# leonsick/depthg

Measured on AMD Instinct MI355X. Metric: correlation-loss steps/sec at B=32,C=384,28x28 (fwd+bwd, per-GPU batch 32), higher is better.
Workload: dtype bf16 (feats) / f16 (code) MFMA inputs, f32 accumulate

## Files before the change

### depthg_amd/_lib.py

```python
import ctypes
import os

_HERE = os.path.dirname(os.path.abspath(__file__))
LIB_PATH = os.environ.get("DEPTHG_LIB") or os.path.join(_HERE, "lib", "libdepthg_hip.so")

DG_OUT_COUNT = 9
DG_OUT_TOTAL = 8
DG_VERSION = 118
DG_POINTWISE, DG_ZERO_CLAMP, DG_STABALIZE, DG_DEPTH_TERM, DG_NEED_GRAD, DG_SHARED_COORDS, DG_IDENTITY_GRID, DG_LINE_GRID, \
    DG_EXACT_MASKS, DG_FEATS_UNIT = (1 << i for i in range(10))
DG_LIN_LAYERNORM, DG_LIN_GELU, DG_LIN_IN_BF16, DG_LIN_OUT_BF16 = 1, 2, 4, 8

class CorrDesc(ctypes.Structure):
    _fields_ = [("B", ctypes.c_int32), ("C", ctypes.c_int32), ("D", ctypes.c_int32), ("h", ctypes.c_int32),
                ("w", ctypes.c_int32), ("S", ctypes.c_int32), ("n_neg", ctypes.c_int32),
                ("depth_h", ctypes.c_int32), ("depth_w", ctypes.c_int32), ("flags", ctypes.c_uint32),
                ("shift_intra", ctypes.c_float), ("shift_inter", ctypes.c_float), ("shift_neg", ctypes.c_float),
                ("shift_depth", ctypes.c_float),
                ("w_intra", ctypes.c_float), ("w_inter", ctypes.c_float), ("w_neg", ctypes.c_float),
                ("w_depth", ctypes.c_float), ("code_h", ctypes.c_int32), ("code_w", ctypes.c_int32)]


class AdamSeg(ctypes.Structure):
    _fields_ = [("param", ctypes.c_void_p), ("grad", ctypes.c_void_p), ("exp_avg", ctypes.c_void_p), ("exp_avg_sq", ctypes.c_void_p),
# ... 84 lines not shown
    "dg_vit_linear_forward": (_I, [vp, vp, vp, f32, vp, vp, vp, vp] + [i32] * 4 + [vp]),
    "dg_depthenc_workspace_bytes": (_SZ, [i32] * 5),
    "dg_depthenc_forward": (_I, [vp] * 12 + [i32] * 8 + [vp, vp, _SZ, vp]),
    "dg_depthenc_backward": (_I, [vp] * 12 + [i32] * 6 + [vp] * 11 + [_SZ, vp]),
    "dg_xattn_workspace_bytes": (_SZ, [i32] * 5),
    "dg_xattn_forward": (_I, [vp] * 3 + [i32] * 5 + [f32, f32, u64, vp, vp, vp, _SZ, vp]),
    "dg_xattn_backward": (_I, [vp] * 6 + [i32] * 5 + [f32, f32, u64, vp, vp, vp, vp, _SZ, vp]),
    "dg_xattn_keep_mask": (_I, [u64] + [i32] * 4 + [f32, vp, vp]),
    "dg_augment_workspace_bytes": (_SZ, [i32] * 3),
    "dg_augment_forward": (_I, [vp] + [i64] * 4 + [vp] * 4 + [i32] * 6 + [vp, vp, vp, _SZ, vp]),
    "dg_batch_prep": (_I, [vp, _SZ, vp, vp, vp] + [i32] * 4 + [vp] * 7),
    "dg_corr_main_kernel_name": (_STR, [cp]),
    "dg_corr_intra_folded": (_I, [cp]),
    "dg_prof_main_span": (_I, [vp]),
    "dg_corr_relaunch_main": (_I, [cp, vp, vp, _SZ, vp]),
}
EXPORTS = list(SIGNATURES)

_lib = None


def load():
    global _lib
    if _lib is not None:
        return _lib
    if not os.path.exists(LIB_PATH):
        raise RuntimeError(
            f"depthg_amd: {LIB_PATH} not found. Build it with `make -C depthg_amd/csrc` "
            "(or `python -c 'import __graft_entry__ as g; g.build()'`). There is no fallback path.")
    lib = ctypes.CDLL(LIB_PATH)
# ... 16 lines not shown
```

### depthg_amd/csrc/dg_api_corr.hip

```cpp
#include "dg_api.h"
#include "dg_corr_args.h"
#include "dg_taps.h"

static unsigned long long* g_prof_span = nullptr;
extern "C" int dg_prof_main_span(void* span) { g_prof_span = static_cast<unsigned long long*>(span); return DG_OK; }

enum class Prep { Small, Dense, General };
enum class Sampler { Plane, ChannelLast };
enum class MainKernel { Small, Corr2, CorrMain };
enum class Depth { None, Job, GsBlocks, GsOwnLaunch };
enum class Hist { Rows, Blobs };
enum class Masks { None, Sampled, DenseRaw, DenseSplit };

struct PairSet {
    int rop;
    int op;
    int neg;
    bool mapped;
    float shift;
    int slot_loss, slot_cd;
    float fin_scale;
    int gidx, csel, dest;
    float factor;
};
// ... 31 lines not shown
    int8_t gr_key[DG_MAX_JOBS], gr_first[DG_MAX_JOBS];
    int32_t gr_nblk[DG_MAX_JOBS];
    size_t nhwc_f[2], nhwc_c[2];
    size_t rows_f[DG_MAX_NEG + 2], rows_c[DG_MAX_NEG + 2];
    size_t op[DG_MAX_NEG + 2], inv[DG_MAX_NEG + 2], colpart[DG_MAX_NEG + 2], bbar[DG_MAX_NEG + 2];
    size_t ccolpart[DG_MAX_NEG + 2], csum[DG_MAX_NEG + 2], bsplit[DG_MAX_NEG + 2];
    size_t rvec[DG_MAX_NEG + 2], rimg[DG_MAX_NEG + 2];
    size_t nz, nzsum;
    size_t dRA[DG_MAX_NEG + 3], dRB[DG_MAX_NEG + 2];
    size_t part[DG_MAX_NEG + 3];
    size_t comb[2], scratch_out, taps, gbuf[DG_MAX_NEG + 2];
    size_t ticket;
    size_t maskbits[DG_MAX_NEG + 2];
    size_t clo[2];
    size_t gr_list, gr_count, gr_rank;
    size_t dRA2[DG_MAX_NEG + 2], dRBs[DG_MAX_NEG + 2], dRB2[DG_MAX_NEG + 2][2], dRBm[DG_MAX_NEG + 2], part4, om;
    size_t total;

    bool small() const { return prep == Prep::Small; }
    bool dense() const { return prep == Prep::Dense; }
    bool plane() const { return sampler == Sampler::Plane; }
    bool has_masks() const { return masks != Masks::None; }
    bool depth_in_gs() const { return depth_run == Depth::GsBlocks || depth_run == Depth::GsOwnLaunch; }
    bool dense_masks() const { return masks == Masks::DenseRaw || masks == Masks::DenseSplit; }
    bool intra_symmetric() const { return !pointwise || fold; }
    const int64_t* batch_map(int k, const int64_t* perms) const {
        return k < 0 ? nullptr : reinterpret_cast<const int64_t*>(reinterpret_cast<uintptr_t>(perms) + (size_t)k * B * sizeof(int64_t));
    }
    const int64_t* map_of(int t, const int64_t* perms) const { return batch_map(ps[t].mapped ? ps[t].neg : -1, perms); }
};
// ... 141 lines not shown
    if ((d->flags & DG_EXACT_MASKS) && p.grad && (d->flags & DG_ZERO_CLAMP) && !xmask && !xmask_dense && !p.small())
        return fail(DG_ERR_UNSUPPORTED, "DG_EXACT_MASKS: exact clamp masks exist on small sample grids (always on there) and on the dense "
                                        "identity grid with C <= 384 (padded to 384), D <= 80, P >= 160, B <= 64, zero_clamp without stabalize");
    p.masks = xmask ? Masks::Sampled : (!xmask_dense ? Masks::None : (p.pointwise ? Masks::DenseSplit : Masks::DenseRaw));
    for (int t = 0; t < p.T; ++t) p.maskbits[t] = take(p.has_masks() ? B * (size_t)(p.Ppad / 32) * p.Ppad * 4 : 0);
    p.main = p.small() ? MainKernel::Small
                       : (p.grad && dg_corr2_shape_supported(p.KF, p.KD, p.D, p.lo, p.hi, p.Ppad, p.B) ? MainKernel::Corr2 : MainKernel::CorrMain);
    static const bool fold_on = [] { const char* e = getenv("DG_FOLD_INTRA"); return !(e && e[0] == '0'); }();
    p.fold = fold_on && p.main == MainKernel::Corr2 && p.pointwise && !xmask;
    p.half = p.main == MainKernel::Corr2 && ident && p.N * p.B <= 512 && p.S == p.h && p.S == p.w;
    p.depth_run = (!p.depth || p.small()) ? Depth::None : (!p.grad ? Depth::Job : (p.dense_masks() ? Depth::GsOwnLaunch : Depth::GsBlocks));
    for (int i = 0; i < 2; ++i) p.clo[i] = take(p.masks == Masks::DenseSplit ? B * (size_t)(p.Ppad / 32) * p.KD * 64 : 0);
    p.gr_list = take((size_t)DG_MAX_JOBS * B * DG_GR_CAP * 4);
    p.gr_count = take((size_t)DG_MAX_JOBS * B * 4);
    p.gr_rank = take((size_t)DG_MAX_JOBS * B * 2);
    {
        const bool sg = p.small() && p.grad, two = sg && p.pointwise;
        const size_t gt = B * p.Ppad * p.KD * 4;
        for (int t = 0; t < p.T; ++t) {
            p.dRA2[t] = take(two ? gt : 0);
            p.dRBs[t] = take(sg && p.nsplit == 2 ? gt : 0);
            for (int k = 0; k < 2; ++k) p.dRB2[t][k] = take(two && k < p.nsplit ? gt : 0);
            p.dRBm[t] = take(sg && t >= 2 && (p.pointwise || p.nsplit == 2) ? gt : 0);
        }
        p.part4 = take(p.small() ? (size_t)(p.T + 1) * B * p.nsplit * 16 : 0);
        p.om = take(p.small() ? (size_t)(p.T + 1) * 4 : 0);
    }
    if (intra_feats) {
        const int x = p.xop = p.T;
        p.nhwc_x = take(rows ? 0 : B * HW * p.C4 * 4);
// ... 341 lines not shown
        f.ext_inv = c.feat_inv ? c.feat_inv + (size_t)o * p.B * p.P : nullptr;
        f.K = p.C; f.K4 = p.C4; f.Kpad = p.KF; f.is_code = 0; f.h = p.h; f.w = p.w;
        DgGatherJob& k = g.jobs[nj++];
        k.src = p.plane() ? f32(c.ws, p.rows_c[o]) : f32(c.ws, p.nhwc_c[srcsel]); k.coords = c.coords(o); k.srcidx = idx;
        k.blob = c.ws + p.op[o]; k.inv_norm = f32(c.ws, p.inv[o]); k.colpart = f32(c.ws, p.ccolpart[o]);
        k.K = p.D; k.K4 = p.D4; k.Kpad = p.KD; k.is_code = 1; k.h = p.hc; k.w = p.wc;
    }
    g.njobs = nj;
    g.direct = p.plane() ? 1 : 0;
    if (p.masks == Masks::Sampled) cd_mask_args(c, p.rows_c, g.cd);
    g.pre = pre_late;
    DG_HIP(dg_launch_gather(g, p.KF, c.stream));
    return DG_OK;
}

static int fwd_colmeans(Fwd& c) {
    const Plan& p = c.p;
    const DgCorrArgs& a = c.a;
    DgColmeanArgs m;
    memset(&m, 0, sizeof(m));
    m.nops = p.nopx(); m.B = p.B; m.P = p.P; m.Ppad = p.Ppad; m.KF = p.KF; m.KD = p.KD;
    for (int o = 0; o < p.nopx(); ++o) {
        m.colpart[o] = p.pointwise ? f32(c.ws, p.colpart[o]) : nullptr; m.bbar[o] = f32(c.ws, p.bbar[o]);
        m.bsplit[o] = reinterpret_cast<__bf16*>(c.ws + p.bsplit[o]);
        m.ngroups[o] = p.Ppad / 32;
        m.ccolpart[o] = f32(c.ws, p.ccolpart[o]); m.csum[o] = f32(c.ws, p.csum[o]);
    }
    m.zero_word = p.depth_in_gs() ? reinterpret_cast<unsigned int*>(c.ws + p.ticket) : nullptr;
    m.zero_words9 = a.wctr;
    if (p.gr_on) {
        m.gr.nh = p.T; m.gr.nkeys = p.gr_nkeys; m.gr.B = p.B;
        for (int t = 0; t < p.T; ++t) { m.gr.sidx[t] = p.map_of(t, c.perms); m.gr.key[t] = p.gr_key[t]; }
        m.gr.list = reinterpret_cast<int32_t*>(c.ws + p.gr_list); m.gr.count = reinterpret_cast<int32_t*>(c.ws + p.gr_count);
        m.gr.rank = reinterpret_cast<int16_t*>(c.ws + p.gr_rank);
    }
    if (p.dense() && p.pointwise) {
        m.dc.code[0] = c.code; m.dc.code[1] = c.code_pos;
        for (int o = 0; o < 2; ++o) { m.dc.blob[o] = c.ws + p.op[o]; m.dc.inv_norm[o] = f32(c.ws, p.inv[o]); m.dc.ccolpart[o] = f32(c.ws, p.ccolpart[o]); }
        m.dc.B = p.B; m.dc.D = p.D; m.dc.KF = p.KF; m.dc.KD = p.KD; m.dc.h = p.h; m.dc.w = p.w; m.dc.P = p.P; m.dc.Ppad = p.Ppad;
        if (p.masks == Masks::DenseSplit) { m.dc.clo[0] = c.ws + p.clo[0]; m.dc.clo[1] = c.ws + p.clo[1]; }
    }
    if (c.split) {
        DgColmeanArgs ms = m;
        ms.zsel = 1; m.zsel = 2;
        DG_HIP(c.side->hand_over(0));
        DG_HIP(dg_launch_colmean(ms, c.side->stream()));
    }
    DG_HIP(dg_launch_colmean(m, c.stream));
    return DG_OK;
}
// ... 219 lines not shown
                f.add(k == 0 ? p.dRB[t] : p.dRBs[t], route, q.gidx, q.csel, q.factor, q.dest, 0);
                if (p.pointwise) f.add(p.dRB2[t][k], route, q.gidx, q.csel, q.factor, q.dest, 0, 0, om);
            }
        }
    }
}

static void scatter_sources_blobs(const Plan& p, const int64_t* perms, ScatterFill& f) {
    const int hf = p.half ? 1 : 0;
    for (int t = 0; t < p.T; ++t) {
        const PairSet& q = p.ps[t];
        const bool doubled = t == 0 && p.intra_symmetric();
        f.add(p.dRA[t], nullptr, q.gidx, 0, doubled ? 2.0f * q.factor : q.factor, 0, 1, hf);
        if (!doubled) f.add(p.dRB[t], p.batch_map(q.neg, perms), q.gidx, q.csel, q.factor, q.dest, 0, hf);
    }
}

static int corr_backward_impl(const dg_corr_desc* desc, const float* grad_scalars, const float* grad_total, const float* coords1,
                              const float* coords2, const int64_t* perms, float* grad_code, float* grad_code_pos,
                              void* workspace, size_t workspace_bytes, dg_stream_t stream_) {
    Plan p{};
    int rc = make_plan(desc, p);
    if (rc != DG_OK) return rc;
    if (!p.grad) return fail(DG_ERR_INVALID, "dg_corr_backward needs a descriptor with DG_NEED_GRAD (as used in forward)");
    if (!coords1 || !coords2 || !grad_code || !grad_code_pos || !workspace) return fail(DG_ERR_INVALID, "null pointer");
    if (p.N > 0 && !perms) return fail(DG_ERR_INVALID, "perms is null with n_neg=%d", p.N);
    if (workspace_bytes < p.total) return fail(DG_ERR_WORKSPACE, "workspace %zu < required %zu bytes", workspace_bytes, p.total);
    char* ws = static_cast<char*>(workspace);
    DgScatterArgs s;
    memset(&s, 0, sizeof(s));
    ScatterFill fill{s, ws};
    if (p.small()) scatter_sources_small(p, perms, fill);
    else scatter_sources_blobs(p, perms, fill);
    if (p.depth) fill.add(p.dRA[p.T], nullptr, 3, 0, 2.0f * p.grad_f, 0, 1);
    s.coords1 = coords1; s.coords2 = coords2; s.gscal = grad_scalars; s.gtot = grad_total;
    s.wtot[0] = desc->w_intra; s.wtot[1] = desc->w_inter; s.wtot[2] = desc->w_neg; s.wtot[3] = desc->w_depth;
    s.comb[0] = f32(ws, p.comb[0]); s.comb[1] = f32(ws, p.comb[1]);
    s.taps = ws + p.taps;
    s.xop = ws + p.op[0]; s.xinv = f32(ws, p.inv[0]); s.blob_bytes = p.blob; s.blob_off_c = p.blob_off_c;
    s.xinv_dest[0] = f32(ws, p.inv[0]); s.xinv_dest[1] = p.nops > 1 ? f32(ws, p.inv[1]) : nullptr;
    s.out[0] = grad_code; s.out[1] = grad_code_pos;
    s.B = p.B; s.D = p.D; s.DP = p.KD; s.h = p.hc; s.w = p.wc; s.S = p.S; s.Sh = p.Sh; s.P = p.P; s.Ppad = p.Ppad;
    if ((size_t)p.hc * p.wc > 4096) return fail(DG_ERR_UNSUPPORTED, "code map %dx%d too large for the gradient gather (max 4096 pixels)", p.hc, p.wc);
    s.DC = 8;
    s.dense = p.dense() ? 1 : 0;
    s.taps_ready = p.dense() ? 0 : 1;
    DG_HIP(dg_launch_scatter(s, static_cast<hipStream_t>(stream_)));
    return DG_OK;
}

extern "C" int dg_corr_backward(const dg_corr_desc* desc, const float* grad_scalars, const float* coords1,
                                const float* coords2, const int64_t* perms, float* grad_code, float* grad_code_pos,
                                void* workspace, size_t workspace_bytes, dg_stream_t stream_) {
    if (!grad_scalars) return fail(DG_ERR_INVALID, "null pointer");
    return corr_backward_impl(desc, grad_scalars, nullptr, coords1, coords2, perms, grad_code, grad_code_pos, workspace,
                              workspace_bytes, stream_);
}

extern "C" int dg_corr_backward_total(const dg_corr_desc* desc, const float* grad_total, const float* coords1,
                                      const float* coords2, const int64_t* perms, float* grad_code, float* grad_code_pos,
// ... 91 lines not shown
    if (!workspace || workspace_bytes < p.total) return fail(DG_ERR_WORKSPACE, "workspace missing or too small");
    if (p.N > 0 && !perms) return fail(DG_ERR_INVALID, "perms is null");
    char* ws = static_cast<char*>(workspace);
    if (p.small()) {
        DgSmallArgs m;
        small_args(p, desc, ws, perms, m);
        m.out = f32(ws, p.scratch_out);
        DG_HIP(dg_launch_corr_small(m, static_cast<hipStream_t>(stream_)));
        return DG_OK;
    }
    DgCorrArgs a;
    build_corr_jobs(p, ws, perms, a);
    return launch_main(p, a, static_cast<hipStream_t>(stream_));
}

extern "C" int dg_corr_intra_folded(const dg_corr_desc* desc) {
    Plan p{};
    if (make_plan(desc, p) != DG_OK) return -1;
    return p.fold ? 1 : 0;
}

extern "C" const char* dg_corr_main_kernel_name(const dg_corr_desc* desc) {
    Plan p{};
    if (make_plan(desc, p) != DG_OK) return nullptr;
    return p.main == MainKernel::Small ? "k_corr_small" : (p.main == MainKernel::Corr2 ? "k_corr2" : "k_corr_main");
}

extern "C" int dg_normalize_split(int32_t B, int32_t C, int32_t h, int32_t w, const float* src, int32_t nchunks, int32_t chunk_c,
                                  float* const* dst, dg_stream_t stream_) {
    if (B < 1 || C < 1 || h < 1 || w < 1 || !src || !dst) return fail(DG_ERR_INVALID, "dg_normalize_split: bad arguments");
// ... 7 lines not shown
```

### depthg_amd/csrc/dg_corr_args.h

```cpp
#pragma once
#include "dg_device.h"

__host__ __device__ inline int dg_perm32(int pl) {
    int s = pl >> 4, u = (pl >> 3) & 1, hh = (pl >> 2) & 1, v = pl & 3;
    return (2 * s + hh) * 8 + 4 * u + v;
}

#ifndef DG_F_IG
#define DG_F_IG 4
#endif
__host__ __device__ inline int dg_f_off(int q, int g) {
    constexpr int IG = DG_F_IG;
    return ((g / IG) * 32 + q) * (IG * 16) + (((g % IG) ^ ((q / (16 / IG)) % IG)) * 16);
}

struct DgBlob {
    int GF, GD, KD;
    int off_c, off_p, bytes;
    __host__ __device__ DgBlob(int KF, int KD_) : GF(KF / 8), GD(KD_ / 8), KD(KD_) {
        off_c = 32 * GF * 16;
        off_p = off_c + GD * 32 * 16;
        bytes = off_p + 4 * KD * 16;
    }
    __host__ __device__ int f(int q, int g) const { return dg_f_off(q, g); }
// ... 9 lines not shown
    static constexpr int BYTES = OFF_P + 4 * KD * 16;
    static constexpr int CHUNKS = BYTES / 1024;
    static constexpr int CHUNK_C0 = OFF_C / 1024;
    static constexpr int CHUNK_P0 = OFF_P / 1024;
    static_assert(BYTES % 1024 == 0 && OFF_C % 1024 == 0 && OFF_P % 1024 == 0, "blob parts must be KiB multiples");
    static_assert(GF % 16 == 0, "swizzle needs 16-granule groups");
};

__host__ __device__ inline size_t dg_gtile_off(int p, int d, int DP) {
    const int q = p & 31;
    return ((size_t)(p >> 5) * (DP >> 5) + (d >> 5)) * 1024 + (q >> 3) * 256 + ((d & 31) + 32 * ((q >> 2) & 1)) * 4 + (q & 3);
}

#define DG_XROWS_LDS (4 * 33 * 16)
template <int NDF>
__device__ __forceinline__ void dg_load_code_rows(const char* Cp, char* T, int lane, _Float16 (&x)[NDF][16]) {
        const int r = lane & 31, h = lane >> 5;
    i32x4 raw[NDF][2];
#pragma unroll
    for (int f = 0; f < NDF; ++f)
#pragma unroll
        for (int k = 0; k < 2; ++k) raw[f][k] = *reinterpret_cast<const i32x4*>(Cp + f * 2048 + k * 1024 + lane * 16);
#pragma unroll
    for (int f = 0; f < NDF; ++f) {
#pragma unroll
        for (int k = 0; k < 2; ++k) {
            const int L = k * 64 + lane;
            *reinterpret_cast<i32x4*>(T + ((L >> 5) * 33 + (L & 31)) * 16) = raw[f][k];
        }
#pragma unroll
        for (int i = 0; i < 16; ++i) {
            const int q = (i & 3) + 8 * (i >> 2) + 4 * h;
            x[f][i] = *reinterpret_cast<const _Float16*>(T + ((r >> 3) * 33 + q) * 16 + (r & 7) * 2);
        }
    }
}

enum { DG_JOB_HELPER = 0, DG_JOB_DEPTH = 1 };

struct DgJob {
    const char* Rop;
    const char* Sop;
    const float* rvec;
    const float* rimg;
    const uint32_t* maskbits;
    const float* nzR;
    const float* nzS;
    const float* RcInv;
    const float* Scsum;
    const int64_t* ridx;
// ... 267 lines not shown
    int cnt = 0;
#pragma unroll
    for (int j = 0; j < DG_MAX_JOBS; ++j) {
        const bool hit = src[j] == m;
        const unsigned long long mask = __ballot(hit);
        if (hit) {
            const int rk = cnt + __popcll(mask & ((1ull << lane) - 1ull));
            g.rank[j * B + lane] = (int16_t)(rk < 32767 ? rk : 32767);
            if (rk < DG_GR_CAP) g.list[(key * B + m) * DG_GR_CAP + rk] = j | (lane << 8);
        }
        cnt += __popcll(mask);
    }
    if (lane == 0) g.count[key * B + m] = cnt < DG_GR_CAP ? cnt : DG_GR_CAP;
}

struct DgColmeanArgs {
    const float* colpart[DG_MAX_NEG + 2];
    float* bbar[DG_MAX_NEG + 2];
    __bf16* bsplit[DG_MAX_NEG + 2];
    const float* ccolpart[DG_MAX_NEG + 2];
    float* csum[DG_MAX_NEG + 2];
    int32_t ngroups[DG_MAX_NEG + 2];
    int32_t nops, B, P, Ppad, KF, KD;
    unsigned int* zero_word;
    unsigned int* zero_words9;
    DgGroupArgs gr;
    DgDenseCodeArgs dc;
    int32_t zsel;
};

struct DgRowmeanJob {
    const char* A;
    const float* bbar;
    const __bf16* bsplit;
    const int64_t* aidx;
    const int64_t* bidx;
    float* rvec;
    float* rimg;
};
struct DgRowmeanArgs {
    DgRowmeanJob jobs[DG_MAX_NEG + 2];
// ... 25 lines not shown
    int32_t nsrc;
    const float* coords1;
    const float* coords2;
    const float* gscal;
    const float* gtot;
    float wtot[4];
    float* comb[2];
    char* taps;
    const char* xop;
    const float* xinv;
    const float* xinv_dest[2];
    int32_t blob_bytes, blob_off_c;
    float* out[2];
    int32_t B, D, DP, h, w, S, Sh, P, Ppad, DC;
    int32_t dense;
    int8_t craw[2][DG_MAX_SCATTER / 2], cfin[2][DG_MAX_SCATTER / 2];
    int8_t ncraw[2], ncfin[2];
    int8_t crawh[2][DG_MAX_SCATTER / 2], cfinh[2][DG_MAX_SCATTER / 2];
    int8_t ncrawh[2], ncfinh[2];
    int32_t routed_half;
    int32_t taps_ready;
    int32_t naxpy;
    float* axo[DG_MAX_NEG + 2];
    const float* axd[DG_MAX_NEG + 2];
    const float* axd2[DG_MAX_NEG + 2];
    const float* axs[DG_MAX_NEG + 2];
    const float* axs2[DG_MAX_NEG + 2];
    const float* axf[DG_MAX_NEG + 2];
};

__device__ __forceinline__ float dg_src_factor(const DgScatterSrc& q) { return q.dfac ? q.factor * q.dfac[0] : q.factor; }
__device__ __forceinline__ float dg_gscal(const DgScatterArgs& a, int i) {
    return a.gscal ? a.gscal[i] + a.gscal[DG_OUT_TOTAL] * a.wtot[i] : a.gtot[0] * a.wtot[i];
}

struct DgGsJob {
    const uint16_t* G;
    const char* Rop;
    const char* Sop;
    const float* ScInv;
    const int64_t* ridx;
    const int64_t* sidx;
    float* dS;
};
struct DgGsArgs {
// ... 64 lines not shown
```

### depthg_amd/csrc/dg_post.hip

```cpp
#include "dg_device.h"
#include "dg_corr_args.h"
#include "dg_taps.h"
#include <cstdlib>

typedef const float __attribute__((address_space(1)))* gfloat_p;


#define DG_LOAD_GS(a, gs)                                                                                   \
    float gs[4];                                                                                            \
    {                                                                                                       \
        const bool vec_ = (a).gscal != nullptr;                                                             \
        const float gt_ = vec_ ? (a).gscal[DG_OUT_TOTAL] : (a).gtot[0];                                     \
        const float g0_ = vec_ ? (a).gscal[0] : 0.f, g1_ = vec_ ? (a).gscal[1] : 0.f;                       \
        const float g2_ = vec_ ? (a).gscal[2] : 0.f, g3_ = vec_ ? (a).gscal[3] : 0.f;                       \
        gs[0] = g0_ + gt_ * (a).wtot[0]; gs[1] = g1_ + gt_ * (a).wtot[1];                                  \
        gs[2] = g2_ + gt_ * (a).wtot[2]; gs[3] = g3_ + gt_ * (a).wtot[3];                                  \
    }
__device__ __forceinline__ float dg_pick(const float (&gs)[4], int i) { return i == 0 ? gs[0] : (i == 1 ? gs[1] : (i == 2 ? gs[2] : gs[3])); }

template <int NDF>
__global__ __launch_bounds__(64 * NDF) void k_grad_combine(const DgScatterArgs a) {
    const int rt = blockIdx.x, n = blockIdx.y, dest = blockIdx.z;
    const int lane = threadIdx.x & 63, r = lane & 31, h = lane >> 5, DP = NDF * 32;
    const int d = __builtin_amdgcn_readfirstlane((int)threadIdx.x >> 6);
// ... 78 lines not shown
        float* out = a.comb[dest] + tile_off;
#pragma unroll
        for (int g = 0; g < 4; ++g) {
            const f32x4 t = {v[4 * g], v[4 * g + 1], v[4 * g + 2], v[4 * g + 3]};
            *reinterpret_cast<f32x4*>(out + g * 256) = t;
        }
    }
}

#ifndef COMB_HB_HM
#define COMB_HB_HM 4
#endif
#ifndef COMB_HB
#define COMB_HB 4
#endif
#define COMB_MAXROUTE 512
template <int NDF, bool HM = false>
__global__ __launch_bounds__(64 * NDF) void k_combine_out(const DgScatterArgs a) {
    const int rt = blockIdx.x, n = blockIdx.y, dest = blockIdx.z;
    const int tid = threadIdx.x, lane = tid & 63, r = lane & 31, h = lane >> 5, DP = NDF * 32;
    const int d = __builtin_amdgcn_readfirstlane(tid >> 6);
    __shared__ __attribute__((aligned(16))) char xs[NDF][DG_XROWS_LDS];
    __shared__ float part[NDF][32];
    __shared__ float stage[NDF][32 * 33];
    __shared__ const float* rl_p[COMB_MAXROUTE];
    __shared__ float rl_w[COMB_MAXROUTE];
    __shared__ int rl_cnt, wcnt[NDF], rsrc[DG_MAX_SCATTER];
    DG_LOAD_GS(a, gs)
    int nr = 0;
    for (int s = 0; s < a.nsrc; ++s)
        if (a.src[s].dest == dest && a.src[s].route != nullptr) { if (tid == 0) rsrc[nr] = s; ++nr; }
    if (tid == 0) rl_cnt = 0;
    __syncthreads();
    for (int i0 = 0; i0 < nr * a.B; i0 += 64 * NDF) {
        const int i = i0 + tid;
        bool hit = false;
        int m = 0, s = 0;
        if (i < nr * a.B) {
            const int rs = i / a.B;
            m = i - rs * a.B; s = rsrc[rs];
            hit = (int)a.src[s].route[m] == n;
        }
        const unsigned long long bal = __ballot(hit);
        if (lane == 0) wcnt[d] = __popcll(bal);
        __syncthreads();
        int base = rl_cnt;
        for (int wv = 0; wv < d; ++wv) base += wcnt[wv];
        if (hit) {
            const int o = base + __popcll(bal & ((1ull << lane) - 1));
            const DgScatterSrc& q = a.src[s];
            if (o < COMB_MAXROUTE) {
                rl_p[o] = q.half ? reinterpret_cast<const float*>(reinterpret_cast<const _Float16*>(q.buf) + (size_t)m * a.Ppad * a.DP) : q.buf + (size_t)m * a.Ppad * a.DP;
                rl_w[o] = dg_src_factor(q) * dg_pick(gs, q.gidx);
            }
        }
        __syncthreads();
        if (tid == 0) {
            int c = rl_cnt;
            for (int wv = 0; wv < NDF; ++wv) c += wcnt[wv];
            rl_cnt = min(c, COMB_MAXROUTE);
        }
        __syncthreads();
    }
    const int cnt = rl_cnt;
    const bool ok = 32 * d + r < a.D;
    const size_t in_img = (size_t)rt * (32 * DP) + lane * 4 + (ok ? d * 1024 : 0);
    const size_t tile_off = (size_t)n * a.Ppad * DP + in_img;
    float v[16];
#pragma unroll
    for (int i = 0; i < 16; ++i) v[i] = 0.f;
    const size_t in_img_h = (size_t)rt * (32 * DP) + lane * 8 + (ok ? d * 1024 : 0);
    constexpr int HB = HM ? COMB_HB_HM : COMB_HB, FB = HM ? 1 : 4;
    float invd[16];
#pragma unroll
    for (int i = 0; i < 16; ++i) {
        const int rr = rt * 32 + (i & 3) + 8 * (i >> 2) + 4 * h;
        invd[i] = (a.xinv_dest[dest] && rr < a.P) ? a.xinv_dest[dest][(size_t)n * a.Ppad + rr] : 0.f;
    }
    const _Float16 __attribute__((address_space(1)))* const hdummy = reinterpret_cast<const _Float16 __attribute__((address_space(1)))*>(reinterpret_cast<uintptr_t>(a.xinv));
// ... 9 lines not shown
            const bool use = ok && sc[u] != 0.f;
#pragma unroll
            for (int e = 0; e < 8; ++e) {
                v[e] = fmaf(raw ? sc[u] : sc[u] * invd[e], use ? (float)t0[u][e] : 0.f, v[e]);
                v[8 + e] = fmaf(raw ? sc[u] : sc[u] * invd[8 + e], use ? (float)t1[u][e] : 0.f, v[8 + e]);
            }
        }
    };
    auto add_sources_half = [&](const int8_t* list, const int nsrc_, const bool raw) __attribute__((always_inline)) {
        for (int k0 = 0; k0 < nsrc_; k0 += HB) {
            const _Float16 __attribute__((address_space(1)))* hb[HB];
            float sc[HB];
#pragma unroll
            for (int u = 0; u < HB; ++u) {
                const bool live = k0 + u < nsrc_;
                const DgScatterSrc& q = a.src[(int)list[live ? k0 + u : k0]];
                sc[u] = live ? dg_src_factor(q) * dg_pick(gs, q.gidx) : 0.f;
                hb[u] = live ? reinterpret_cast<const _Float16 __attribute__((address_space(1)))*>(reinterpret_cast<uintptr_t>(q.buf)) + (size_t)n * a.Ppad * DP + in_img_h
                             : hdummy;
            }
            add_half4(hb, sc, raw);
        }
    };
    auto add_sources = [&](const int8_t* list, const int nsrc_) __attribute__((always_inline)) {

        for (int k0 = 0; k0 < nsrc_; k0 += FB) {
            f32x4 t[FB][4];
            float sc[FB];
#pragma unroll
            for (int u = 0; u < FB; ++u) {
                const bool live = k0 + u < nsrc_;
                const DgScatterSrc& q = a.src[(int)list[live ? k0 + u : k0]];
                sc[u] = live ? dg_src_factor(q) * dg_pick(gs, q.gidx) : 0.f;
                const float* base = q.buf + tile_off;
#pragma unroll
                for (int g = 0; g < 4; ++g) t[u][g] = *reinterpret_cast<const f32x4*>(base + (ok ? g * 256 : 0));
            }
#pragma unroll
            for (int u = 0; u < FB; ++u) {
                const bool use = ok && k0 + u < nsrc_;
#pragma unroll
                for (int g = 0; g < 4; ++g)
#pragma unroll
                    for (int e = 0; e < 4; ++e) v[4 * g + e] = fmaf(sc[u], use ? t[u][g][e] : 0.f, v[4 * g + e]);
            }
        }
    };
    const int nraw = a.ncraw[dest] + a.ncrawh[dest];
    add_sources(a.craw[dest], a.ncraw[dest]);
    add_sources_half(a.crawh[dest], a.ncrawh[dest], true);
    if (nraw > 0) {
        const char* xb = a.xop + ((size_t)n * (a.Ppad >> 5) + rt) * a.blob_bytes + a.blob_off_c + d * 2048;
        _Float16 x[1][16];
        dg_load_code_rows<1>(xb, xs[d], lane, x);
#pragma unroll
        for (int i = 0; i < 16; ++i) {
            const float t = half_sum((float)x[0][i] * v[i]);
            if (r == 0) part[d][h * 16 + i] = t;
        }
        __syncthreads();
#pragma unroll
        for (int i = 0; i < 16; ++i) {
            float t = part[0][h * 16 + i];
#pragma unroll
            for (int f = 1; f < NDF; ++f) t += part[f][h * 16 + i];
            const int rr = rt * 32 + (i & 3) + 8 * (i >> 2) + 4 * h;
            const float inv = rr < a.P ? a.xinv[(size_t)n * a.Ppad + rr] : 0.f;
            v[i] = (v[i] - (float)x[0][i] * t) * inv;
        }
    }
    add_sources(a.cfin[dest], a.ncfin[dest]);
    add_sources_half(a.cfinh[dest], a.ncfinh[dest], false);
    if (a.routed_half) {
        for (int e0 = 0; e0 < cnt; e0 += HB) {
            const _Float16 __attribute__((address_space(1)))* hb[HB];
            float sc[HB];
#pragma unroll
            for (int k = 0; k < HB; ++k) {
                const int e = min(e0 + k, cnt - 1);
                sc[k] = e0 + k < cnt ? rl_w[e] : 0.f;
                hb[k] = sc[k] != 0.f ? reinterpret_cast<const _Float16 __attribute__((address_space(1)))*>(reinterpret_cast<uintptr_t>(rl_p[e])) + in_img_h : hdummy;
            }
            add_half4(hb, sc, false);
        }
    } else
    for (int e0 = 0; e0 < cnt; e0 += 4) {
        f32x4 u4[4][4];
        float sc[4];
#pragma unroll
        for (int k = 0; k < 4; ++k) {
            const int e = min(e0 + k, cnt - 1);
            sc[k] = e0 + k < cnt ? rl_w[e] : 0.f;
            const gfloat_p sb = (gfloat_p)rl_p[e] + in_img;
#pragma unroll
            for (int g = 0; g < 4; ++g) u4[k][g] = *(const f32x4 __attribute__((address_space(1)))*)(sb + (ok ? g * 256 : 0));
        }
#pragma unroll
        for (int k = 0; k < 4; ++k)
#pragma unroll
            for (int g = 0; g < 4; ++g)
#pragma unroll
                for (int e = 0; e < 4; ++e) v[4 * g + e] = fmaf(sc[k], ok ? u4[k][g][e] : 0.f, v[4 * g + e]);
    }
    float* st = stage[d];
#pragma unroll
    for (int i = 0; i < 16; ++i) st[r * 33 + (i & 3) + 8 * (i >> 2) + 4 * h] = v[i];
    __builtin_amdgcn_fence(__ATOMIC_RELEASE, "workgroup");
    __builtin_amdgcn_wave_barrier();
// ... 363 lines not shown
    for (int c = 0; c < CG; ++c) {
        const int d = 32 * f + CG * cg + c;
        if (d >= a.D) break;
        for (int pix = tid; pix < HW; pix += DENSE_THREADS) out[((size_t)b * a.D + d) * HW + pix] = stage[c * (HW + 1) + pix];
    }
}

hipError_t dg_launch_scatter(const DgScatterArgs& a, hipStream_t s) {
    DgScatterArgs ac = a;
    {
        for (int dest = 0; dest < 2; ++dest) {
            ac.ncraw[dest] = ac.ncfin[dest] = ac.ncrawh[dest] = ac.ncfinh[dest] = 0;
            for (int i = 0; i < a.nsrc; ++i) {
                const DgScatterSrc& q = a.src[i];
                if (q.dest != dest || q.route != nullptr) continue;
                int8_t& cnt = q.half ? (q.raw ? ac.ncrawh[dest] : ac.ncfinh[dest]) : (q.raw ? ac.ncraw[dest] : ac.ncfin[dest]);
                if (cnt >= DG_MAX_SCATTER / 2) return hipErrorInvalidValue;
                (q.half ? (q.raw ? ac.crawh[dest] : ac.cfinh[dest]) : (q.raw ? ac.craw[dest] : ac.cfin[dest]))[cnt++] = (int8_t)i;
            }
        }
        const dim3 cgrid(a.Ppad / 32, a.B, 2);
        {
            int nrouted = 0;
            for (int i = 0; i < a.nsrc; ++i) nrouted += a.src[i].route != nullptr;
            bool any_half = false;
            int routed_h = 0;
            for (int i = 0; i < a.nsrc; ++i) { any_half = any_half || a.src[i].half != 0; routed_h += (a.src[i].route != nullptr && a.src[i].half) ? 1 : 0; }
            if (routed_h != 0 && routed_h != nrouted) return hipErrorInvalidValue;
            ac.routed_half = routed_h != 0 ? 1 : 0;
            const bool one_launch = a.dense && a.S == a.h && a.S == a.w && nrouted * a.B <= COMB_MAXROUTE && (a.DP == 96 || a.DP == 128);
            if (any_half && !one_launch) return hipErrorInvalidValue;
            if (one_launch) {
                if (a.DP == 96 && any_half) hipLaunchKernelGGL((k_combine_out<3, true>), cgrid, dim3(192), 0, s, ac);
                else if (a.DP == 96) hipLaunchKernelGGL(k_combine_out<3>, cgrid, dim3(192), 0, s, ac);
                else hipLaunchKernelGGL(k_combine_out<4>, cgrid, dim3(256), 0, s, ac);
                return hipGetLastError();
            }
        }
        const dim3 cgrid2(a.Ppad / 32, a.B, 2 + a.naxpy);
        if (a.DP == 96) hipLaunchKernelGGL(k_grad_combine<3>, cgrid2, dim3(192), 0, s, ac);
        else if (a.DP == 128) hipLaunchKernelGGL(k_grad_combine<4>, cgrid2, dim3(256), 0, s, ac);
        else return hipErrorInvalidValue;
    }
    const int HW = a.h * a.w;
    {
        int nrouted = 0;
        for (int i = 0; i < a.nsrc; ++i) nrouted += a.src[i].route != nullptr;
// ... 321 lines not shown
```

### depthg_amd/csrc/dg_prep.hip

```cpp
#include "dg_device.h"
#include "dg_corr_args.h"
#include "dg_taps.h"
#include <cstdlib>

__global__ void k_nchw_to_nhwc(const DgTransposeArgs a) {
    __shared__ float t[32][33];
    const int b = blockIdx.z;
    int m = 0, gy = blockIdx.y;
    while (m < a.nmaps - 1 && gy >= (a.K4[m] + 31) / 32) { gy -= (a.K4[m] + 31) / 32; ++m; }
    const float* __restrict__ src = a.src[m];
    float* __restrict__ dst = a.dst[m];
    const int K = a.K[m], K4 = a.K4[m], HW = a.HW[m];
    const int k0 = gy * 32, p0 = blockIdx.x * 32;
    if (p0 >= HW) return;
    const int tx = threadIdx.x, ty = threadIdx.y;
    for (int i = ty; i < 32; i += 8) {
        int k = k0 + i, p = p0 + tx;
        t[i][tx] = (k < K && p < HW) ? src[((size_t)b * K + k) * HW + p] : 0.f;
    }
    __syncthreads();
    for (int i = ty; i < 32; i += 8) {
        int p = p0 + i, k = k0 + tx;
        if (p < HW && k < K4) dst[((size_t)b * HW + p) * K4 + k] = t[tx][i];
    }
// ... 917 lines not shown
    const int n = blockIdx.x, o = blockIdx.y;
    if (a.zero_word && n == 0 && o == 0 && blockIdx.z == 0 && threadIdx.x == 0) *a.zero_word = 0u;
    if (a.zero_words9 && n == 0 && o == 0 && blockIdx.z == 0 && threadIdx.x < 9) a.zero_words9[threadIdx.x] = 0u;
    auto reduce = [&](const float* part, int ngroups, int K, float scale, float* out) __attribute__((always_inline)) { colsum_reduce(part, n, ngroups, K, scale, out); };
    if (a.zsel == 1 ? blockIdx.z != 3 : (a.zsel == 2 && blockIdx.z == 3)) return;
    if (blockIdx.z == 3) {
        const int GD = a.dc.KD / 8;
        if ((int)blockIdx.y < 2 * GD) dense_code_planes(a.dc, cm_smem, n, (int)blockIdx.y / GD, (int)blockIdx.y % GD);
        return;
    }
    if (blockIdx.z == 2) {
        if ((int)blockIdx.y < a.gr.nkeys && threadIdx.x < 64) dg_group_lists(a.gr, n, o, threadIdx.x);
        return;
    }
    if (o >= a.nops) return;
    if (blockIdx.z == 0 && a.colpart[o]) {
        reduce(a.colpart[o], a.ngroups[o], a.KF, 1.f / (float)a.P, a.bbar[o]);
        __syncthreads();
        for (int k = threadIdx.x; k < a.KF; k += 256) {
            const float v = a.bbar[o][(size_t)n * a.KF + k];
            const __bf16 hi = (__bf16)v;
            a.bsplit[o][((size_t)n * 2) * a.KF + k] = hi;
            a.bsplit[o][((size_t)n * 2 + 1) * a.KF + k] = (__bf16)(v - (float)hi);
        }
    }
    if (blockIdx.z == 1 && a.ccolpart[o] && a.dc.B == 0) reduce(a.ccolpart[o], a.Ppad / 32, a.KD, 1.f, a.csum[o]);
}

hipError_t dg_launch_colmean(const DgColmeanArgs& a, hipStream_t s) {
    int ny = a.gr.nkeys > a.nops ? a.gr.nkeys : a.nops;
    int nz = a.gr.nkeys > 0 ? 3 : 2, smem = 0;
    if (a.dc.B > 0) {
        if (a.nops != 2) return hipErrorInvalidValue;
        ny = max(ny, 2 * (a.dc.KD / 8)); nz = 4; smem = a.dc.Ppad * 16 * ((a.dc.clo[0] || a.dc.clo[1]) ? 2 : 1);
    }
    return dg_launch_if(a.dc.B > 0, k_colmean, dim3(a.B, ny, nz), dim3(256), smem, s, a);
}

#define ROWMEAN_WAVES 4
template <bool XJ = false>
__global__ __launch_bounds__(64 * ROWMEAN_WAVES) void k_rowmean(const DgRowmeanArgs a) {
    extern __shared__ __attribute__((aligned(16))) char rm_smem[];
    const int tile = blockIdx.x, n = blockIdx.y, tid = threadIdx.x, lane = tid & 63, c = lane & 31, h = lane >> 5;
    const int wid = __builtin_amdgcn_readfirstlane(tid >> 6);
    const int KF = a.KF, nt = a.Ppad / 32;
    const bool xz = XJ && blockIdx.z == 1;
// ... 105 lines not shown
```

### include/depthg_corr.h

```cpp
#ifndef DEPTHG_CORR_H
#define DEPTHG_CORR_H

#include <stddef.h>
#include <stdint.h>

#ifdef __cplusplus
extern "C" {
#endif

#define DG_VERSION 118

#define DG_POINTWISE      (1u << 0)
#define DG_ZERO_CLAMP     (1u << 1)
#define DG_STABALIZE      (1u << 2)
#define DG_DEPTH_TERM     (1u << 3)
#define DG_NEED_GRAD      (1u << 4)
#define DG_SHARED_COORDS  (1u << 5)

#define DG_IDENTITY_GRID  (1u << 6)

#define DG_LINE_GRID      (1u << 7)

#define DG_EXACT_MASKS    (1u << 8)

// ... 321 lines not shown
#define DG_BATCH_MASK_BOOL_IGNORED   0
#define DG_BATCH_MASK_FLOAT_POSITIVE 1
int dg_batch_prep(const uint8_t* packed, size_t packed_bytes, const int32_t* records_host, const int32_t* tables_host,
                  const void* params, int32_t n_records, int32_t N, int32_t H, int32_t W, const float* mean, const float* stdv,
                  float* img, int64_t* label, void* mask, float* depth, dg_stream_t stream);

const char* dg_corr_main_kernel_name(const dg_corr_desc* desc);

int dg_corr_intra_folded(const dg_corr_desc* desc);

int dg_prof_main_span(void* span);

int dg_corr_relaunch_main(const dg_corr_desc* desc, const int64_t* perms,
                          void* workspace, size_t workspace_bytes, dg_stream_t stream);

#ifdef __cplusplus
}
#endif
#endif
```

Baseline: 3348.

## Precompute routed scatter lists in colmean kernel instead of per-block in combine

Inverse-permutation route lists for the combine kernel are now built once per image in the forward colmean launch and stored in workspace. The backward combine kernel then reads the ready list instead of scanning all routed sources with ballots and several barriers in every block. The change also issues the code-row global loads early so they overlap the raw source accumulation, and reuses already-loaded inverse norms when they match. It adds a workspace buffer, a new API export, and a dependency between the forward and backward passes on that buffer.

Measured after the change: 3380 (median of 6 runs). Within noise of the previous version (+1.0%).

```diff
diff --git a/depthg_amd/_lib.py b/depthg_amd/_lib.py
--- a/depthg_amd/_lib.py
+++ b/depthg_amd/_lib.py
@@ -122,6 +122,7 @@
     "dg_corr_intra_folded": (_I, [cp]),
     "dg_prof_main_span": (_I, [vp]),
     "dg_corr_relaunch_main": (_I, [cp, vp, vp, _SZ, vp]),
+    "dg_corr_route_table": (_I, [cp, vp, vp, vp, vp]),
 }
 EXPORTS = list(SIGNATURES)
 
diff --git a/depthg_amd/csrc/dg_api_corr.hip b/depthg_amd/csrc/dg_api_corr.hip
--- a/depthg_amd/csrc/dg_api_corr.hip
+++ b/depthg_amd/csrc/dg_api_corr.hip
@@ -69,6 +69,8 @@
     size_t maskbits[DG_MAX_NEG + 2];
     size_t clo[2];
     size_t gr_list, gr_count, gr_rank;
+    int rt_cap, rt_slots;
+    size_t rt_list, rt_count;
     size_t dRA2[DG_MAX_NEG + 2], dRBs[DG_MAX_NEG + 2], dRB2[DG_MAX_NEG + 2][2], dRBm[DG_MAX_NEG + 2], part4, om;
     size_t total;
 
@@ -240,6 +242,10 @@
     p.gr_list = take((size_t)DG_MAX_JOBS * B * DG_GR_CAP * 4);
     p.gr_count = take((size_t)DG_MAX_JOBS * B * 4);
     p.gr_rank = take((size_t)DG_MAX_JOBS * B * 2);
+    p.rt_cap = (ident && p.grad && p.N > 0 && (size_t)p.N * B <= COMB_MAXROUTE) ? p.N * p.B : 0;
+    p.rt_slots = p.rt_cap > 0 ? 1 : 0;
+    p.rt_list = take((size_t)p.rt_slots * B * p.rt_cap * 4);
+    p.rt_count = take((size_t)p.rt_slots * B * 4);
     {
         const bool sg = p.small() && p.grad, two = sg && p.pointwise;
         const size_t gt = B * p.Ppad * p.KD * 4;
@@ -611,6 +617,8 @@
     return DG_OK;
 }
 
+static void route_args(const Plan& p, char* ws, const int64_t* perms, DgRouteArgs& r);
+
 static int fwd_colmeans(Fwd& c) {
     const Plan& p = c.p;
     const DgCorrArgs& a = c.a;
@@ -631,6 +639,7 @@
         m.gr.list = reinterpret_cast<int32_t*>(c.ws + p.gr_list); m.gr.count = reinterpret_cast<int32_t*>(c.ws + p.gr_count);
         m.gr.rank = reinterpret_cast<int16_t*>(c.ws + p.gr_rank);
     }
+    if (p.rt_cap > 0) route_args(p, c.ws, c.perms, m.rt);
     if (p.dense() && p.pointwise) {
         m.dc.code[0] = c.code; m.dc.code[1] = c.code_pos;
         for (int o = 0; o < 2; ++o) { m.dc.blob[o] = c.ws + p.op[o]; m.dc.inv_norm[o] = f32(c.ws, p.inv[o]); m.dc.ccolpart[o] = f32(c.ws, p.ccolpart[o]); }
@@ -880,6 +889,23 @@
         f.add(p.dRA[t], nullptr, q.gidx, 0, doubled ? 2.0f * q.factor : q.factor, 0, 1, hf);
         if (!doubled) f.add(p.dRB[t], p.batch_map(q.neg, perms), q.gidx, q.csel, q.factor, q.dest, 0, hf);
     }
+}
+
+static void route_args(const Plan& p, char* ws, const int64_t* perms, DgRouteArgs& r) {
+    DgScatterArgs s;
+    memset(&s, 0, sizeof(s));
+    ScatterFill fill{s, ws};
+    scatter_sources_blobs(p, perms, fill);
+    for (int i = 0; i < s.nsrc; ++i) {
+        const DgScatterSrc& q = s.src[i];
+        if (!q.route) continue;
+        const int k = r.nr[q.dest]++;
+        r.map[q.dest][k] = q.route; r.src[q.dest][k] = (int8_t)i;
+    }
+    int nslot = 0;
+    for (int d = 0; d < 2; ++d) r.slot[d] = r.nr[d] > 0 ? (int8_t)nslot++ : (int8_t)-1;
+    r.B = p.B; r.cap = p.rt_cap; r.slots = p.rt_slots;
+    r.list = reinterpret_cast<int32_t*>(ws + p.rt_list); r.count = reinterpret_cast<int32_t*>(ws + p.rt_count);
 }
 
 static int corr_backward_impl(const dg_corr_desc* desc, const float* grad_scalars, const float* grad_total, const float* coords1,
@@ -910,6 +936,10 @@
     if ((size_t)p.hc * p.wc > 4096) return fail(DG_ERR_UNSUPPORTED, "code map %dx%d too large for the gradient gather (max 4096 pixels)", p.hc, p.wc);
     s.DC = 8;
     s.dense = p.dense() ? 1 : 0;
+    if (p.rt_cap > 0) {
+        s.rt_list = reinterpret_cast<const int32_t*>(ws + p.rt_list); s.rt_count = reinterpret_cast<const int32_t*>(ws + p.rt_count);
+        s.rt_cap = p.rt_cap; s.rt_slots = p.rt_slots;
+    }
     s.taps_ready = p.dense() ? 0 : 1;
     DG_HIP(dg_launch_scatter(s, static_cast<hipStream_t>(stream_)));
     return DG_OK;
@@ -1031,6 +1061,14 @@
     return launch_main(p, a, static_cast<hipStream_t>(stream_));
 }
 
+extern "C" int dg_corr_route_table(const dg_corr_desc* desc, size_t* list_offset, size_t* count_offset, int32_t* cap, int32_t* slots) {
+    Plan p{};
+    if (int rc = make_plan(desc, p)) return rc;
+    if (!list_offset || !count_offset || !cap || !slots) return fail(DG_ERR_INVALID, "dg_corr_route_table: null pointer");
+    *list_offset = p.rt_list; *count_offset = p.rt_count; *cap = p.rt_cap; *slots = p.rt_slots;
+    return DG_OK;
+}
+
 extern "C" int dg_corr_intra_folded(const dg_corr_desc* desc) {
     Plan p{};
     if (make_plan(desc, p) != DG_OK) return -1;
diff --git a/depthg_amd/csrc/dg_corr_args.h b/depthg_amd/csrc/dg_corr_args.h
--- a/depthg_amd/csrc/dg_corr_args.h
+++ b/depthg_amd/csrc/dg_corr_args.h
@@ -47,13 +47,15 @@
 
 #define DG_XROWS_LDS (4 * 33 * 16)
 template <int NDF>
-__device__ __forceinline__ void dg_load_code_rows(const char* Cp, char* T, int lane, _Float16 (&x)[NDF][16]) {
-        const int r = lane & 31, h = lane >> 5;
-    i32x4 raw[NDF][2];
+__device__ __forceinline__ void dg_code_rows_fetch(const char* Cp, int lane, i32x4 (&raw)[NDF][2]) {
 #pragma unroll
     for (int f = 0; f < NDF; ++f)
 #pragma unroll
         for (int k = 0; k < 2; ++k) raw[f][k] = *reinterpret_cast<const i32x4*>(Cp + f * 2048 + k * 1024 + lane * 16);
+}
+template <int NDF>
+__device__ __forceinline__ void dg_code_rows_turn(const i32x4 (&raw)[NDF][2], char* T, int lane, _Float16 (&x)[NDF][16]) {
+    const int r = lane & 31, h = lane >> 5;
 #pragma unroll
     for (int f = 0; f < NDF; ++f) {
 #pragma unroll
@@ -67,6 +69,12 @@
             x[f][i] = *reinterpret_cast<const _Float16*>(T + ((r >> 3) * 33 + q) * 16 + (r & 7) * 2);
         }
     }
+}
+template <int NDF>
+__device__ __forceinline__ void dg_load_code_rows(const char* Cp, char* T, int lane, _Float16 (&x)[NDF][16]) {
+    i32x4 raw[NDF][2];
+    dg_code_rows_fetch<NDF>(Cp, lane, raw);
+    dg_code_rows_turn<NDF>(raw, T, lane, x);
 }
 
 enum { DG_JOB_HELPER = 0, DG_JOB_DEPTH = 1 };
@@ -364,6 +372,38 @@
     if (lane == 0) g.count[key * B + m] = cnt < DG_GR_CAP ? cnt : DG_GR_CAP;
 }
 
+#define COMB_MAXROUTE 512
+struct DgRouteArgs {
+    const int64_t* map[2][DG_MAX_NEG];
+    int8_t src[2][DG_MAX_NEG];
+    int8_t nr[2];
+    int8_t slot[2];
+    int32_t B, cap, slots;
+    int32_t* list;
+    int32_t* count;
+};
+__device__ __forceinline__ void dg_route_lists(const DgRouteArgs& g, const int dest, const int n, const int lane) {
+    const int B = g.B, nr = g.nr[dest];
+    int first[DG_MAX_NEG];
+#pragma unroll
+    for (int k = 0; k < DG_MAX_NEG; ++k) first[k] = (k < nr && lane < B) ? (int)g.map[dest][k][lane] : -1;
+    int32_t* const row = g.list + ((size_t)g.slot[dest] * B + n) * g.cap;
+    int cnt = 0;
+#pragma unroll
+    for (int k = 0; k < DG_MAX_NEG; ++k) {
+        if (k >= nr) break;
+        for (int m0 = 0; m0 < B; m0 += 64) {
+            const int m = m0 + lane;
+            const int to = m0 == 0 ? first[k] : (m < B ? (int)g.map[dest][k][m] : -1);
+            const bool hit = to == n;
+            const unsigned long long mask = __ballot(hit);
+            if (hit) row[cnt + __popcll(mask & ((1ull << lane) - 1ull))] = (int)g.src[dest][k] | (m << 8);
+            cnt += __popcll(mask);
+        }
+    }
+    if (lane == 0) g.count[g.slot[dest] * B + n] = cnt;
+}
+
 struct DgColmeanArgs {
     const float* colpart[DG_MAX_NEG + 2];
     float* bbar[DG_MAX_NEG + 2];
@@ -375,6 +415,7 @@
     unsigned int* zero_word;
     unsigned int* zero_words9;
     DgGroupArgs gr;
+    DgRouteArgs rt;
     DgDenseCodeArgs dc;
     int32_t zsel;
 };
@@ -430,11 +471,15 @@
     float* out[2];
     int32_t B, D, DP, h, w, S, Sh, P, Ppad, DC;
     int32_t dense;
-    int8_t craw[2][DG_MAX_SCATTER / 2], cfin[2][DG_MAX_SCATTER / 2];
-    int8_t ncraw[2], ncfin[2];
-    int8_t crawh[2][DG_MAX_SCATTER / 2], cfinh[2][DG_MAX_SCATTER / 2];
-    int8_t ncrawh[2], ncfinh[2];
+    alignas(4) int8_t craw[2][DG_MAX_SCATTER / 2], cfin[2][DG_MAX_SCATTER / 2];
+    int32_t ncraw[2], ncfin[2];
+    alignas(4) int8_t crawh[2][DG_MAX_SCATTER / 2], cfinh[2][DG_MAX_SCATTER / 2];
+    int32_t ncrawh[2], ncfinh[2];
     int32_t routed_half;
+    const int32_t* rt_list;
+    const int32_t* rt_count;
+    int32_t rt_cap, rt_slots;
+    int32_t rt_nr[2], rt_slot[2];
     int32_t taps_ready;
     int32_t naxpy;
     float* axo[DG_MAX_NEG + 2];
@@ -445,6 +490,10 @@
     const float* axf[DG_MAX_NEG + 2];
 };
 
+static_assert(sizeof(DgScatterArgs) <= 4096 && (DG_MAX_SCATTER / 2) % 4 == 0, "the argument block of a launch holds 4 KiB; the source lists are read by words");
+__device__ __forceinline__ int dg_list_at(const int8_t* list, int i) {
+    return (reinterpret_cast<const int32_t*>(list)[i >> 2] >> ((i & 3) * 8)) & 0xff;
+}
 __device__ __forceinline__ float dg_src_factor(const DgScatterSrc& q) { return q.dfac ? q.factor * q.dfac[0] : q.factor; }
 __device__ __forceinline__ float dg_gscal(const DgScatterArgs& a, int i) {
     return a.gscal ? a.gscal[i] + a.gscal[DG_OUT_TOTAL] * a.wtot[i] : a.gtot[0] * a.wtot[i];
diff --git a/depthg_amd/csrc/dg_post.hip b/depthg_amd/csrc/dg_post.hip
--- a/depthg_amd/csrc/dg_post.hip
+++ b/depthg_amd/csrc/dg_post.hip
@@ -116,7 +116,6 @@
 #ifndef COMB_HB
 #define COMB_HB 4
 #endif
-#define COMB_MAXROUTE 512
 template <int NDF, bool HM = false>
 __global__ __launch_bounds__(64 * NDF) void k_combine_out(const DgScatterArgs a) {
     const int rt = blockIdx.x, n = blockIdx.y, dest = blockIdx.z;
@@ -125,46 +124,29 @@
     __shared__ __attribute__((aligned(16))) char xs[NDF][DG_XROWS_LDS];
     __shared__ float part[NDF][32];
     __shared__ float stage[NDF][32 * 33];
-    __shared__ const float* rl_p[COMB_MAXROUTE];
-    __shared__ float rl_w[COMB_MAXROUTE];
-    __shared__ int rl_cnt, wcnt[NDF], rsrc[DG_MAX_SCATTER];
+    constexpr int NT = 64 * NDF, RLR = (COMB_MAXROUTE + NT - 1) / NT;
+    __shared__ int rl_e[RLR * NT];
+    __shared__ float sw[DG_MAX_SCATTER];
     DG_LOAD_GS(a, gs)
-    int nr = 0;
-    for (int s = 0; s < a.nsrc; ++s)
-        if (a.src[s].dest == dest && a.src[s].route != nullptr) { if (tid == 0) rsrc[nr] = s; ++nr; }
-    if (tid == 0) rl_cnt = 0;
-    __syncthreads();
-    for (int i0 = 0; i0 < nr * a.B; i0 += 64 * NDF) {
-        const int i = i0 + tid;
-        bool hit = false;
-        int m = 0, s = 0;
-        if (i < nr * a.B) {
-            const int rs = i / a.B;
-            m = i - rs * a.B; s = rsrc[rs];
-            hit = (int)a.src[s].route[m] == n;
-        }
-        const unsigned long long bal = __ballot(hit);
-        if (lane == 0) wcnt[d] = __popcll(bal);
-        __syncthreads();
-        int base = rl_cnt;
-        for (int wv = 0; wv < d; ++wv) base += wcnt[wv];
-        if (hit) {
-            const int o = base + __popcll(bal & ((1ull << lane) - 1));
-            const DgScatterSrc& q = a.src[s];
-            if (o < COMB_MAXROUTE) {
-                rl_p[o] = q.half ? reinterpret_cast<const float*>(reinterpret_cast<const _Float16*>(q.buf) + (size_t)m * a.Ppad * a.DP) : q.buf + (size_t)m * a.Ppad * a.DP;
-                rl_w[o] = dg_src_factor(q) * dg_pick(gs, q.gidx);
-            }
-        }
-        __syncthreads();
-        if (tid == 0) {
-            int c = rl_cnt;
-            for (int wv = 0; wv < NDF; ++wv) c += wcnt[wv];
-            rl_cnt = min(c, COMB_MAXROUTE);
-        }
-        __syncthreads();
-    }
-    const int cnt = rl_cnt;
+    const int nrd = a.rt_nr[dest];
+    const int slot = a.rt_slot[dest];
+    const int cnt = nrd > 0 ? min(a.rt_count[slot * a.B + n], a.rt_cap) : 0;
+    int ent[RLR];
+#pragma unroll
+    for (int k = 0; k < RLR; ++k) ent[k] = 0;
+    float s_fac = 0.f;
+    int s_gi = 0;
+    gfloat_p s_df = nullptr;
+    if (nrd > 0) {
+        const int32_t* const row = a.rt_list + ((size_t)slot * a.B + n) * a.rt_cap;
+#pragma unroll
+        for (int k = 0; k < RLR; ++k) ent[k] = row[min(k * NT + tid, a.rt_cap - 1)];
+        const DgScatterSrc& q = a.src[min(tid, a.nsrc - 1)];
+        s_fac = q.factor; s_gi = q.gidx; s_df = (gfloat_p)q.dfac;
+    }
+    const int nraw = a.ncraw[dest] + a.ncrawh[dest];
+    i32x4 xraw[1][2] = {};
+    if (nraw > 0) dg_code_rows_fetch<1>(a.xop + ((size_t)n * (a.Ppad >> 5) + rt) * a.blob_bytes + a.blob_off_c + d * 2048, lane, xraw);
     const bool ok = 32 * d + r < a.D;
     const size_t in_img = (size_t)rt * (32 * DP) + lane * 4 + (ok ? d * 1024 : 0);
     const size_t tile_off = (size_t)n * a.Ppad * DP + in_img;
@@ -204,7 +186,7 @@
 #pragma unroll
             for (int u = 0; u < HB; ++u) {
                 const bool live = k0 + u < nsrc_;
-                const DgScatterSrc& q = a.src[(int)list[live ? k0 + u : k0]];
+                const DgScatterSrc& q = a.src[dg_list_at(list, live ? k0 + u : k0)];
                 sc[u] = live ? dg_src_factor(q) * dg_pick(gs, q.gidx) : 0.f;
                 hb[u] = live ? reinterpret_cast<const _Float16 __attribute__((address_space(1)))*>(reinterpret_cast<uintptr_t>(q.buf)) + (size_t)n * a.Ppad * DP + in_img_h
                              : hdummy;
@@ -213,14 +195,13 @@
         }
     };
     auto add_sources = [&](const int8_t* list, const int nsrc_) __attribute__((always_inline)) {
-
         for (int k0 = 0; k0 < nsrc_; k0 += FB) {
             f32x4 t[FB][4];
             float sc[FB];
 #pragma unroll
             for (int u = 0; u < FB; ++u) {
                 const bool live = k0 + u < nsrc_;
-                const DgScatterSrc& q = a.src[(int)list[live ? k0 + u : k0]];
+                const DgScatterSrc& q = a.src[dg_list_at(list, live ? k0 + u : k0)];
                 sc[u] = live ? dg_src_factor(q) * dg_pick(gs, q.gidx) : 0.f;
                 const float* base = q.buf + tile_off;
 #pragma unroll
@@ -236,28 +217,34 @@
             }
         }
     };
-    const int nraw = a.ncraw[dest] + a.ncrawh[dest];
     add_sources(a.craw[dest], a.ncraw[dest]);
     add_sources_half(a.crawh[dest], a.ncrawh[dest], true);
+    if (nrd > 0) {
+#pragma unroll
+        for (int k = 0; k < RLR; ++k) rl_e[k * NT + tid] = ent[k];
+        if (tid < a.nsrc) sw[tid] = (s_df ? s_fac * s_df[0] : s_fac) * dg_pick(gs, s_gi);
+    }
     if (nraw > 0) {
-        const char* xb = a.xop + ((size_t)n * (a.Ppad >> 5) + rt) * a.blob_bytes + a.blob_off_c + d * 2048;
         _Float16 x[1][16];
-        dg_load_code_rows<1>(xb, xs[d], lane, x);
+        dg_code_rows_turn<1>(xraw, xs[d], lane, x);
 #pragma unroll
         for (int i = 0; i < 16; ++i) {
             const float t = half_sum((float)x[0][i] * v[i]);
             if (r == 0) part[d][h * 16 + i] = t;
         }
         __syncthreads();
+        const bool same_inv = a.xinv_dest[dest] == a.xinv;
 #pragma unroll
         for (int i = 0; i < 16; ++i) {
             float t = part[0][h * 16 + i];
 #pragma unroll
             for (int f = 1; f < NDF; ++f) t += part[f][h * 16 + i];
             const int rr = rt * 32 + (i & 3) + 8 * (i >> 2) + 4 * h;
-            const float inv = rr < a.P ? a.xinv[(size_t)n * a.Ppad + rr] : 0.f;
+            const float inv = same_inv ? invd[i] : (rr < a.P ? a.xinv[(size_t)n * a.Ppad + rr] : 0.f);
             v[i] = (v[i] - (float)x[0][i] * t) * inv;
         }
+    } else if (nrd > 0) {
+        __syncthreads();
     }
     add_sources(a.cfin[dest], a.ncfin[dest]);
     add_sources_half(a.cfinh[dest], a.ncfinh[dest], false);
@@ -267,9 +254,10 @@
             float sc[HB];
 #pragma unroll
             for (int k = 0; k < HB; ++k) {
-                const int e = min(e0 + k, cnt - 1);
-                sc[k] = e0 + k < cnt ? rl_w[e] : 0.f;
-                hb[k] = sc[k] != 0.f ? reinterpret_cast<const _Float16 __attribute__((address_space(1)))*>(reinterpret_cast<uintptr_t>(rl_p[e])) + in_img_h : hdummy;
+                const int en = __builtin_amdgcn_readfirstlane(rl_e[min(e0 + k, cnt - 1)]), s = min(en & 255, a.nsrc - 1), m = min((en >> 8) & 0xffff, a.B - 1);
+                sc[k] = e0 + k < cnt ? sw[s] : 0.f;
+                hb[k] = sc[k] != 0.f ? reinterpret_cast<const _Float16 __attribute__((address_space(1)))*>(reinterpret_cast<uintptr_t>(a.src[s].buf)) + (size_t)m * a.Ppad * a.DP + in_img_h
+                                     : hdummy;
             }
             add_half4(hb, sc, false);
         }
@@ -279,9 +267,9 @@
         float sc[4];
 #pragma unroll
         for (int k = 0; k < 4; ++k) {
-            const int e = min(e0 + k, cnt - 1);
-            sc[k] = e0 + k < cnt ? rl_w[e] : 0.f;
-            const gfloat_p sb = (gfloat_p)rl_p[e] + in_img;
+            const int en = __builtin_amdgcn_readfirstlane(rl_e[min(e0 + k, cnt - 1)]), s = min(en & 255, a.nsrc - 1), m = min((en >> 8) & 0xffff, a.B - 1);
+            sc[k] = e0 + k < cnt ? sw[s] : 0.f;
+            const gfloat_p sb = (gfloat_p)a.src[s].buf + (size_t)m * a.Ppad * a.DP + in_img;
 #pragma unroll
             for (int g = 0; g < 4; ++g) u4[k][g] = *(const f32x4 __attribute__((address_space(1)))*)(sb + (ok ? g * 256 : 0));
         }
@@ -675,7 +663,7 @@
             for (int i = 0; i < a.nsrc; ++i) {
                 const DgScatterSrc& q = a.src[i];
                 if (q.dest != dest || q.route != nullptr) continue;
-                int8_t& cnt = q.half ? (q.raw ? ac.ncrawh[dest] : ac.ncfinh[dest]) : (q.raw ? ac.ncraw[dest] : ac.ncfin[dest]);
+                int32_t& cnt = q.half ? (q.raw ? ac.ncrawh[dest] : ac.ncfinh[dest]) : (q.raw ? ac.ncraw[dest] : ac.ncfin[dest]);
                 if (cnt >= DG_MAX_SCATTER / 2) return hipErrorInvalidValue;
                 (q.half ? (q.raw ? ac.crawh[dest] : ac.cfinh[dest]) : (q.raw ? ac.craw[dest] : ac.cfin[dest]))[cnt++] = (int8_t)i;
             }
@@ -692,6 +680,13 @@
             const bool one_launch = a.dense && a.S == a.h && a.S == a.w && nrouted * a.B <= COMB_MAXROUTE && (a.DP == 96 || a.DP == 128);
             if (any_half && !one_launch) return hipErrorInvalidValue;
             if (one_launch) {
+                ac.rt_nr[0] = ac.rt_nr[1] = 0;
+                for (int i = 0; i < a.nsrc; ++i)
+                    if (a.src[i].route != nullptr) { if (a.src[i].dest < 0 || a.src[i].dest > 1) return hipErrorInvalidValue; ++ac.rt_nr[a.src[i].dest]; }
+                const int nrmax = ac.rt_nr[0] > ac.rt_nr[1] ? ac.rt_nr[0] : ac.rt_nr[1];
+                int nslot = 0;
+                for (int dd = 0; dd < 2; ++dd) ac.rt_slot[dd] = ac.rt_nr[dd] > 0 ? nslot++ : -1;
+                if (nrmax > 0 && (!a.rt_list || !a.rt_count || nrmax * a.B > a.rt_cap || a.rt_cap > COMB_MAXROUTE || nslot > a.rt_slots)) return hipErrorInvalidValue;
                 if (a.DP == 96 && any_half) hipLaunchKernelGGL((k_combine_out<3, true>), cgrid, dim3(192), 0, s, ac);
                 else if (a.DP == 96) hipLaunchKernelGGL(k_combine_out<3>, cgrid, dim3(192), 0, s, ac);
                 else hipLaunchKernelGGL(k_combine_out<4>, cgrid, dim3(256), 0, s, ac);
diff --git a/depthg_amd/csrc/dg_prep.hip b/depthg_amd/csrc/dg_prep.hip
--- a/depthg_amd/csrc/dg_prep.hip
+++ b/depthg_amd/csrc/dg_prep.hip
@@ -955,6 +955,7 @@
         return;
     }
     if (o >= a.nops) return;
+    if (blockIdx.z == 1 && a.rt.list && o < 2 && a.rt.nr[o] > 0 && (threadIdx.x >> 6) == 1) dg_route_lists(a.rt, o, n, threadIdx.x & 63);
     if (blockIdx.z == 0 && a.colpart[o]) {
         reduce(a.colpart[o], a.ngroups[o], a.KF, 1.f / (float)a.P, a.bbar[o]);
         __syncthreads();
@@ -971,6 +972,12 @@
 hipError_t dg_launch_colmean(const DgColmeanArgs& a, hipStream_t s) {
     int ny = a.gr.nkeys > a.nops ? a.gr.nkeys : a.nops;
     int nz = a.gr.nkeys > 0 ? 3 : 2, smem = 0;
+    if (a.rt.list) {
+        const int nrmax = a.rt.nr[0] > a.rt.nr[1] ? a.rt.nr[0] : a.rt.nr[1];
+        if (a.rt.B != a.B || a.nops < 2 || nrmax > DG_MAX_NEG || nrmax * a.rt.B > a.rt.cap || a.rt.cap > COMB_MAXROUTE || !a.rt.count) return hipErrorInvalidValue;
+        for (int d = 0; d < 2; ++d)
+            if ((a.rt.nr[d] > 0) != (a.rt.slot[d] >= 0) || a.rt.slot[d] >= a.rt.slots) return hipErrorInvalidValue;
+    }
     if (a.dc.B > 0) {
         if (a.nops != 2) return hipErrorInvalidValue;
         ny = max(ny, 2 * (a.dc.KD / 8)); nz = 4; smem = a.dc.Ppad * 16 * ((a.dc.clo[0] || a.dc.clo[1]) ? 2 : 1);
diff --git a/include/depthg_corr.h b/include/depthg_corr.h
--- a/include/depthg_corr.h
+++ b/include/depthg_corr.h
@@ -359,6 +359,8 @@
 int dg_corr_relaunch_main(const dg_corr_desc* desc, const int64_t* perms,
                           void* workspace, size_t workspace_bytes, dg_stream_t stream);
 
+int dg_corr_route_table(const dg_corr_desc* desc, size_t* list_offset, size_t* count_offset, int32_t* cap, int32_t* slots);
+
 #ifdef __cplusplus
 }
 #endif
```
